# paLeziart/quadruped-reactive-walking

Hardware: AMD Instinct MI355X
Metric: control-steps/sec (MPC+WBC) (higher is better)
Workload: dtype f64

## Files before the change

### quadruped-reactive-walking_amd/csrc/chain_sweep.h

```cpp
#pragma once
#include <hip/hip_runtime.h>

#include "qrw_device.h"

namespace qrw {

constexpr int kCol = 14;
constexpr int kSlot = 168;
__host__ __device__ constexpr int chain_gap(int m) { return 0; }
__host__ __device__ constexpr int chain_slot(int slot, int m) { return slot * kSlot + (slot >= m ? chain_gap(m) : 0); }
__device__ __forceinline__ int chain_row_t(int lane) {
  const int l = lane & 15;
  return (l < 12) ? l : 11;
}
__host__ __device__ constexpr int chain_lds_doubles(int slots, int m) { return slots * kSlot + chain_gap(m); }

__device__ __forceinline__ double dpp_step12(double r, double x, const double (&m)[12]) {
  double a0 = r;
  asm("s_nop 1\n\t"
      "v_fmac_f64_dpp %0, %1, %2 row_newbcast:0 row_mask:0xf bank_mask:0xf\n\t"
      "v_fmac_f64_dpp %0, %1, %3 row_newbcast:1 row_mask:0xf bank_mask:0xf\n\t"
      "v_fmac_f64_dpp %0, %1, %4 row_newbcast:2 row_mask:0xf bank_mask:0xf\n\t"
      "v_fmac_f64_dpp %0, %1, %5 row_newbcast:3 row_mask:0xf bank_mask:0xf\n\t"
      "v_fmac_f64_dpp %0, %1, %6 row_newbcast:4 row_mask:0xf bank_mask:0xf\n\t"
      "v_fmac_f64_dpp %0, %1, %7 row_newbcast:5 row_mask:0xf bank_mask:0xf\n\t"
      "v_fmac_f64_dpp %0, %1, %8 row_newbcast:6 row_mask:0xf bank_mask:0xf\n\t"
      "v_fmac_f64_dpp %0, %1, %9 row_newbcast:7 row_mask:0xf bank_mask:0xf\n\t"
      "v_fmac_f64_dpp %0, %1, %10 row_newbcast:8 row_mask:0xf bank_mask:0xf\n\t"
      "v_fmac_f64_dpp %0, %1, %11 row_newbcast:9 row_mask:0xf bank_mask:0xf\n\t"
      "v_fmac_f64_dpp %0, %1, %12 row_newbcast:10 row_mask:0xf bank_mask:0xf\n\t"
      "v_fmac_f64_dpp %0, %1, %13 row_newbcast:11 row_mask:0xf bank_mask:0xf\n\t"
      : "+v"(a0)
      : "v"(x), "v"(m[0]), "v"(m[1]), "v"(m[2]), "v"(m[3]), "v"(m[4]), "v"(m[5]), "v"(m[6]), "v"(m[7]), "v"(m[8]),
        "v"(m[9]), "v"(m[10]), "v"(m[11]));
  return a0;
}

__host__ __device__ __forceinline__ int chain_pos(int k, int m, int N) { return (k <= m) ? k : m + N - k; }

struct ChainOp {
  double m[12];
  double r;
};
typedef double qrw_d2 __attribute__((ext_vector_type(2)));

__device__ __forceinline__ double swap_halves(double v) {
  int lo = __double2loint(v), hi = __double2hiint(v);
  asm("s_nop 1\n\tv_permlane32_swap_b32 %0, %0\n\tv_permlane32_swap_b32 %1, %1" : "+v"(lo), "+v"(hi));
  return __hiloint2double(hi, lo);
}

__device__ __forceinline__ double swap_rows16(double v) {
  int lo = __double2loint(v), hi = __double2hiint(v);
  asm("s_nop 1\n\tv_permlane16_swap_b32 %0, %0\n\tv_permlane16_swap_b32 %1, %1" : "+v"(lo), "+v"(hi));
  return __hiloint2double(hi, lo);
}

template <int NC>
__device__ __forceinline__ void chain_forward_paired(const double* sN, double* sX, double* sDump, int lane) {
  constexpr int N = NC, m = N >> 1, LA = m, LB = N - 1 - m, NP = LA / 2;
  static_assert(LA % 2 == 0 && LB == LA - 1, "paired sweeps need an even chain length");
  const int i = ((lane & 15) < 12) ? (lane & 15) : 11;
  const int h = lane >> 5;
  const bool rw = (lane & 16) != 0;
  const bool own = (lane & 15) < 12;
  const double* pm = sN + (rw ? m * kSlot + chain_gap(m) : 0) + h * kSlot + i;
  double* px = sX + (rw ? (m + 1) * 12 : 0) + i;
  const double* pr = px + h * 12;
  double* dump = sDump + i;
  double* ps_odd = (own && h == 1) ? px : dump;
  double* ps_even = (own && h == 0) ? px : dump;
  double* ps_oddA = (own && h == 1 && !rw) ? px : dump;
  double x = px[0], pB = 0.0;
  ChainOp b0, b1;
  auto fetch = [&](ChainOp& b, int p) {
    const double* q = pm + 2 * p * kSlot;
#pragma unroll
    for (int c = 0; c < 12; c++) b.m[c] = __hip_atomic_load(q + c * kCol, __ATOMIC_RELAXED, __HIP_MEMORY_SCOPE_WAVEFRONT);
    b.r = pr[(2 * p + 1) * 12];
  };
  auto pair = [&](const ChainOp& b, int p) {
    const int t1 = 2 * p + 1, t2 = t1 + 1;
    x = dpp_step12(b.r, x, b.m);
    x = swap_halves(x);
    if (t1 == LB) pB = x;
    (t1 < LB ? ps_odd : ps_oddA)[t1 * 12] = x;
    x = dpp_step12(b.r, x, b.m);
    if (t2 < LA) {
      x = swap_halves(x);
      ps_even[t2 * 12] = x;
    }
  };
  fetch(b0, 0);
#pragma unroll
  for (int p = 0; p < NP; p += 2) {
    if (p + 1 < NP) fetch(b1, p + 1);
    __builtin_amdgcn_sched_barrier(0);
    pair(b0, p);
    if (p + 1 < NP) {
      if (p + 2 < NP) fetch(b0, p + 2);
      __builtin_amdgcn_sched_barrier(0);
      pair(b1, p + 1);
    }
  }
  x += swap_rows16(pB);
  if (lane >= 32 && lane < 44) sX[m * 12 + i] = x;
}
template <int NC>
__device__ __forceinline__ void chain_backward_paired(const double* sN, double* sX, double* sDump, int lane) {
  constexpr int N = NC, m = N >> 1, LA = m, LB = N - 1 - m, NP = LA / 2;
  static_assert(LA % 2 == 0 && LB == LA - 1, "paired sweeps need an even chain length");
  const int i = ((lane & 15) < 12) ? (lane & 15) : 11;
  const int h = lane >> 5;
  const bool rw = (lane & 16) != 0;
  const bool own = (lane & 15) < 12;
  const int ib = chain_row_t(lane);
  const double* pm = sN + ((rw ? (N - 1) : m) - LA - h) * kSlot + (rw ? chain_gap(m) : 0) + ib * kCol;
  double* px = sX + ((rw ? N : m) - LA) * 12 + i;
  const double* pr = px - h * 12;
  double* dump = sDump + i;
  double* ps_odd = (own && h == 1) ? px : dump;
  double* ps_even = (own && h == 0) ? px : dump;
  double* ps_lastA = (own && h == 1 && !rw) ? px : dump;
  double x = sX[m * 12 + i];
  ChainOp b0, b1;
  auto fetch = [&](ChainOp& b, int p) {
    const qrw_d2* q = reinterpret_cast<const qrw_d2*>(pm + (LA - 2 * p - 1) * kSlot);
#pragma unroll
    for (int c = 0; c < 6; c++) {
      const qrw_d2 v = q[c];
      b.m[2 * c] = v.x;
      b.m[2 * c + 1] = v.y;
    }
    b.r = pr[(LA - 2 * p - 1) * 12];
  };
  auto pair = [&](const ChainOp& b, int p) {
    const int t1 = 2 * p + 1, t2 = t1 + 1;
    x = dpp_step12(b.r, x, b.m);
    x = swap_halves(x);
    ps_odd[(LA - t1) * 12] = x;
    x = dpp_step12(b.r, x, b.m);
    if (t2 < LA) {
      x = swap_halves(x);
      ps_even[(LA - t2) * 12] = x;
    } else {
      ps_lastA[(LA - t2) * 12] = x;
    }
  };
  fetch(b0, 0);
#pragma unroll
  for (int p = 0; p < NP; p += 2) {
    if (p + 1 < NP) fetch(b1, p + 1);
    __builtin_amdgcn_sched_barrier(0);
    pair(b0, p);
    if (p + 1 < NP) {
      if (p + 2 < NP) fetch(b0, p + 2);
      __builtin_amdgcn_sched_barrier(0);
      pair(b1, p + 1);
    }
  }
}

template <int NC>
__device__ __forceinline__ void chain_forward(const double* sN, double* sX, double* sDump, int Nrt, int lane) {
  if constexpr (NC > 0 && (NC / 2) % 2 == 0) {
    chain_forward_paired<NC>(sN, sX, sDump, lane);
    return;
  }
  const int N = NC ? NC : Nrt;
  const int m = N >> 1, LA = m, LB = N - 1 - m;
  if (LA == 0) return;
  asm volatile("" : "+v"(lane));
  const int i = ((lane & 15) < 12) ? (lane & 15) : 11;
  const bool rw = (lane & 16) != 0;
  const bool wr = (lane < 32) && ((lane & 15) < 12);
  const double* pm = sN + (rw ? m * kSlot + chain_gap(m) : 0) + i;
  double* px = sX + (rw ? (m + 1) * 12 : 0) + i;
  double* ps_early = wr ? px : sDump + i;
  double* ps_late = (wr && !rw) ? px : sDump + i;
  double x = px[0], pB = 0.0;
  ChainOp b0, b1;
  auto fetch = [&](ChainOp& b, int t) {
    const double* q = pm + (t - 1) * kSlot;
#pragma unroll
    for (int c = 0; c < 12; c++) {
      b.m[c] = __hip_atomic_load(q + c * kCol, __ATOMIC_RELAXED, __HIP_MEMORY_SCOPE_WAVEFRONT);
    }
    b.r = px[t * 12];
  };
  auto step = [&](const ChainOp& b, int t) {
    x = dpp_step12(b.r, x, b.m);
    if (t == LB) pB = x;
    if (t < LA) (t < LB ? ps_early : ps_late)[t * 12] = x;
  };
  fetch(b0, 1);
#pragma unroll
  for (int t = 1; t <= LA; t += 2) {
    if (t + 1 <= LA) fetch(b1, t + 1);
    __builtin_amdgcn_sched_barrier(0);
    step(b0, t);
    if (t + 1 <= LA) {
      if (t + 2 <= LA) fetch(b0, t + 2);
      __builtin_amdgcn_sched_barrier(0);
      step(b1, t + 1);
    }
  }
  if (LB > 0) x += shfl(pB, lane + 16);
  if (lane < 12) sX[m * 12 + i] = x;
}
template <int NC>
__device__ __forceinline__ void chain_backward(const double* sN, double* sX, double* sDump, int Nrt, int lane) {
  if constexpr (NC > 0 && (NC / 2) % 2 == 0) {
    chain_backward_paired<NC>(sN, sX, sDump, lane);
    return;
  }
  const int N = NC ? NC : Nrt;
  const int m = N >> 1, LA = m, LB = N - 1 - m;
  if (LA == 0) return;
  asm volatile("" : "+v"(lane));
  const int i = ((lane & 15) < 12) ? (lane & 15) : 11;
  const bool rw = (lane & 16) != 0;
  const bool wr = (lane < 32) && ((lane & 15) < 12);
  const int ib = chain_row_t(lane);
  const double* pm = sN + ((rw ? (N - 1) : m) - LA) * kSlot + (rw ? chain_gap(m) : 0) + ib * kCol;
  double* px = sX + ((rw ? N : m) - LA) * 12 + i;
  double* ps_early = wr ? px : sDump + i;
  double* ps_late = (wr && !rw) ? px : sDump + i;
  double x = sX[m * 12 + i];
  ChainOp b0, b1;
  auto fetch = [&](ChainOp& b, int t) {
    const qrw_d2* q = reinterpret_cast<const qrw_d2*>(pm + (LA - t) * kSlot);
#pragma unroll
    for (int c = 0; c < 6; c++) {
      const qrw_d2 v = q[c];
      b.m[2 * c] = v.x;
      b.m[2 * c + 1] = v.y;
    }
    b.r = px[(LA - t) * 12];
  };
  auto step = [&](const ChainOp& b, int t) {
    x = dpp_step12(b.r, x, b.m);
    (t <= LB ? ps_early : ps_late)[(LA - t) * 12] = x;
  };
  fetch(b0, 1);
#pragma unroll
  for (int t = 1; t <= LA; t += 2) {
    if (t + 1 <= LA) fetch(b1, t + 1);
    __builtin_amdgcn_sched_barrier(0);
    step(b0, t);
    if (t + 1 <= LA) {
      if (t + 2 <= LA) fetch(b0, t + 2);
      __builtin_amdgcn_sched_barrier(0);
      step(b1, t + 1);
    }
  }
}

#define QRW_GJ_FM(C) "v_fmac_f64_dpp %" #C ", %" #C ", %12 row_newbcast:%13 row_mask:0xf bank_mask:0xf\n\t"
template <int P>
__device__ __forceinline__ void gj_pivot(double (&m)[12], int i) {
  double piv = 0.0;
  const double one = 1.0;
  asm("s_nop 1\n\tv_fmac_f64_dpp %0, %1, %2 row_newbcast:%3 row_mask:0xf bank_mask:0xf" : "+v"(piv) : "v"(m[P]), "v"(one), "n"(P));
  const double d = fast_rcp(piv);
  const double f = (i == P) ? (d - 1.0) : (-m[P] * d);
  asm("s_nop 1\n\t" QRW_GJ_FM(0) QRW_GJ_FM(1) QRW_GJ_FM(2) QRW_GJ_FM(3) QRW_GJ_FM(4) QRW_GJ_FM(5) QRW_GJ_FM(6) QRW_GJ_FM(7)
      QRW_GJ_FM(8) QRW_GJ_FM(9) QRW_GJ_FM(10) QRW_GJ_FM(11)
      : "+v"(m[0]), "+v"(m[1]), "+v"(m[2]), "+v"(m[3]), "+v"(m[4]), "+v"(m[5]), "+v"(m[6]), "+v"(m[7]), "+v"(m[8]),
        "+v"(m[9]), "+v"(m[10]), "+v"(m[11])
      : "v"(f), "n"(P));
  m[P] = (i == P) ? d : f;
}
#undef QRW_GJ_FM
__device__ __forceinline__ void gj_invert12(double (&m)[12], int i) {
  gj_pivot<0>(m, i); gj_pivot<1>(m, i); gj_pivot<2>(m, i); gj_pivot<3>(m, i); gj_pivot<4>(m, i); gj_pivot<5>(m, i);
  gj_pivot<6>(m, i); gj_pivot<7>(m, i); gj_pivot<8>(m, i); gj_pivot<9>(m, i); gj_pivot<10>(m, i); gj_pivot<11>(m, i);
}
template <int J>
__device__ __forceinline__ void row_bcast_fma(double (&acc)[12], const double (&m)[12], double coef) {
  asm("s_nop 1\n\t"
      "v_fmac_f64_dpp %0, %12, %24 row_newbcast:%25 row_mask:0xf bank_mask:0xf\n\t"
      "v_fmac_f64_dpp %1, %13, %24 row_newbcast:%25 row_mask:0xf bank_mask:0xf\n\t"
      "v_fmac_f64_dpp %2, %14, %24 row_newbcast:%25 row_mask:0xf bank_mask:0xf\n\t"
      "v_fmac_f64_dpp %3, %15, %24 row_newbcast:%25 row_mask:0xf bank_mask:0xf\n\t"
      "v_fmac_f64_dpp %4, %16, %24 row_newbcast:%25 row_mask:0xf bank_mask:0xf\n\t"
      "v_fmac_f64_dpp %5, %17, %24 row_newbcast:%25 row_mask:0xf bank_mask:0xf\n\t"
      "v_fmac_f64_dpp %6, %18, %24 row_newbcast:%25 row_mask:0xf bank_mask:0xf\n\t"
      "v_fmac_f64_dpp %7, %19, %24 row_newbcast:%25 row_mask:0xf bank_mask:0xf\n\t"
      "v_fmac_f64_dpp %8, %20, %24 row_newbcast:%25 row_mask:0xf bank_mask:0xf\n\t"
      "v_fmac_f64_dpp %9, %21, %24 row_newbcast:%25 row_mask:0xf bank_mask:0xf\n\t"
      "v_fmac_f64_dpp %10, %22, %24 row_newbcast:%25 row_mask:0xf bank_mask:0xf\n\t"
      "v_fmac_f64_dpp %11, %23, %24 row_newbcast:%25 row_mask:0xf bank_mask:0xf\n\t"
      : "+v"(acc[0]), "+v"(acc[1]), "+v"(acc[2]), "+v"(acc[3]), "+v"(acc[4]), "+v"(acc[5]), "+v"(acc[6]), "+v"(acc[7]),
        "+v"(acc[8]), "+v"(acc[9]), "+v"(acc[10]), "+v"(acc[11])
      : "v"(m[0]), "v"(m[1]), "v"(m[2]), "v"(m[3]), "v"(m[4]), "v"(m[5]), "v"(m[6]), "v"(m[7]), "v"(m[8]), "v"(m[9]),
        "v"(m[10]), "v"(m[11]), "v"(coef), "n"(J));
}
__device__ __forceinline__ double row_shr6(double v) {
  int lo = __double2loint(v), hi = __double2hiint(v);
  lo = __builtin_amdgcn_update_dpp(0, lo, 0x116, 0xF, 0xF, false);
  hi = __builtin_amdgcn_update_dpp(0, hi, 0x116, 0xF, 0xF, false);
  return __hiloint2double(hi, lo);
}

}
```

### quadruped-reactive-walking_amd/csrc/mpc_kernel.hip

```cpp
#include <hip/hip_runtime.h>
#include <math.h>
#include <stdint.h>

#include <type_traits>
#include <vector>

#include "chain_sweep.h"
#include "qrw_device.h"
#include "qrw_kernels.h"

namespace qrw {

namespace {

constexpr int kMatSz = 144;
constexpr int kWSz = 36;

template <int NW>
struct alignas(16) MpcLdsT {
  static constexpr int S = 16 * NW;
  double sN[chain_lds_doubles(S, S / 2)];
  double sX[(S + 2) * 12];
  double sDump[(S / 2 + 2) * 12];
  double sE[S * 12];
// ... 1230 lines not shown
#ifdef QRW_TRACE_RES
        if (tid == 0 && a.prof && iter <= 4000) {
          double* tr = a.prof + (size_t)b * kMpcProfItems + (iter / 200 - 1) * 3;
          tr[0] = pri_res / (eps_abs + eps_rel * last_np); tr[1] = dua_res / (eps_abs + eps_rel * last_nd); tr[2] = rho;
        }
#endif
        if constexpr (PRE) {
          if (iter - it_resume >= a.pre_chunk && iter < max_iter) {
            if (pre_may_park<NW>(a, &L.sBal[0], tid)) parked = true;
            else it_resume = iter;
          }
          if (tid == 0) {
            double* pr = &L.sPre[(iter / 200 & 1) * 4];
            pr[0] = pri_res; pr[1] = last_np; pr[2] = dua_res; pr[3] = last_nd;
          }
        }
      }
      PH(7);
      if constexpr (PRE) {
        if (parked) break;
      }
    }
  }
  PH(7);
#ifdef QRW_PROFILE_PHASES
  if (tid == 0 && a.prof) for (int i = 0; i < 10; i++) a.prof[(size_t)b * kMpcProfItems + i] = (double)ph_acc[i];
#endif
  if (iter > max_iter) iter = max_iter;
  if (status == kStatusUnsolved && !parked) {
    const bool pok = pri_res < 10.0 * eps_abs + 10.0 * eps_rel * last_np;
    const bool dok = dua_res < 10.0 * eps_abs + 10.0 * eps_rel * last_nd;
    status = (pok && dok) ? kStatusSolvedInaccurate : kStatusMaxIter;
  }

  {
  QRW_UNPARK()
  const bool has_sol = (status != kStatusNonCvx);
  if (act && !parked) {
#pragma unroll
    for (int t = 0; t < 3; t++) {
      const int i = 3 * j + t;
      const double sx = has_sol ? xhX[t] + xr[i * (N + 1) + k + 1] : nan("");
      const double sf = has_sol ? xhF[t] : nan("");
      outp[i * N + k] = sx;
      outp[(12 + i) * N + k] = sf;
    }
  }
#pragma unroll
  for (int t = 0; t < 3; t++) {
    xX[t] = parked ? xhX[t] : xhX[t] * iDx[t]; xF[t] = parked ? xhF[t] : xhF[t] * iDf[t];
    zD[t] = Ed[t] * uD0[t];
    yD[t] = parked ? thD[t] : (thD[t] + zeU[t]) * (1.0 / Ed[t]);
    yS[t] = parked ? etS[t] : etS[t] * (1.0 / Es[t]);
  }
#pragma unroll
  for (int c = 0; c < 5; c++) {
    zC[c] = parked ? zeC[c] : zeC[c] * (1.0 / (rho_used * Ec[c]));
    yC[c] = parked ? etC[c] : etC[c] * (1.0 / Ec[c]);
  }
  if (!has_sol) {
#pragma unroll
    for (int t = 0; t < 3; t++) xX[t] = xF[t] = zD[t] = yD[t] = yS[t] = 0.0;
#pragma unroll
    for (int c = 0; c < 5; c++) zC[c] = yC[c] = 0.0;
  }
  ST(kStRho) = rho;
  ST(kStC) = parked ? rho_used : cs;
#pragma unroll
  for (int t = 0; t < 3; t++) {
    ST(kStXX + t) = xX[t]; ST(kStXF + t) = xF[t]; ST(kStZD + t) = zD[t];
    ST(kStYD + t) = yD[t]; ST(kStYS + t) = yS[t]; ST(kStS + t) = sfl[t];
    ST(kStDX + t) = 1.0 / iDx[t]; ST(kStDF + t) = 1.0 / iDf[t]; ST(kStED + t) = Ed[t]; ST(kStES + t) = Es[t];
#pragma unroll
    for (int r = 0; r < 3; r++) ST(kStB + r * 3 + t) = Bang[r][t];
  }
#pragma unroll
  for (int c = 0; c < 5; c++) { ST(kStZC + c) = zC[c]; ST(kStYC + c) = yC[c]; ST(kStEC + c) = Ec[c]; }
  if (PRE && parked) {
    if (tid == 0) {
      a.pause_it[b] = iter;
      a.rho_updates[b] = rho_updates;
    }
  } else if (tid == 0) {
    if constexpr (PRE) a.pause_it[b] = 0;
    a.flags[b] = 1;
    a.iters[b] = iter;
    a.status[b] = status;
    a.rho_out[b] = rho;
    a.pri[b] = pri_res;
    a.dua[b] = dua_res;
    a.rho_updates[b] = rho_updates;
    if (SEQ && a.seq_iters) a.seq_iters[io] = iter;
#ifdef QRW_SEQ_STATS
    if (a.prof && a.seq_K <= 5) {
      a.prof[io * 2] = (double)(__builtin_amdgcn_s_memrealtime() - task_t0);
      a.prof[io * 2 + 1] = (double)iter;
    }
#endif
  }
  }
  }
  if constexpr (SEQ) seq_finish_task<NW>(a, b, seq_s, tid);
  if constexpr (PRE) {
    int level = 0;
    if (parked && tid == 0) {
      const int it = a.pause_it[b];
      const double* p1 = &L.sPre[(it / 200 & 1) * 4];
      const double* p0 = &L.sPre[((it / 200 & 1) ^ 1) * 4];
      const double r1 = fmax(p1[0] / (1e-6 + 1e-6 * p1[1]), p1[2] / (1e-6 + 1e-6 * p1[3]));
      const double r0 = (p0[1] > 0.0 || p0[3] > 0.0) ? fmax(p0[0] / (1e-6 + 1e-6 * p0[1]), p0[2] / (1e-6 + 1e-6 * p0[3])) : 0.0;
      level = pre_level(a, it, it_resume, r1, r0);
    }
    pre_end_chunk<NW>(a, b, parked, level, tid);
  }
  }
#undef QRW_UNPARK
#undef ST
}

namespace {
__device__ __forceinline__ int order_key(float e) {
  const int key = (int)(e * 0.04f);
  return key < 0 ? 0 : (key > 160 ? 160 : key);
}
__device__ __forceinline__ float order_ema(float e0, float it) { return (e0 == 0.0f) ? it : e0 + (it - e0) * 0.125f; }
}

__global__ __launch_bounds__(64) void mpc_order_kernel(const int* __restrict__ iters, float* __restrict__ ema,
                                                       int* __restrict__ order, int B) {
  constexpr int U = 4, R = 64 * 4 * U;
  __shared__ int hist[162];
  __shared__ int offs[162];
  const int lane = threadIdx.x;
  for (int i = lane; i < 162; i += 64) hist[i] = 0;
  __syncthreads();
  const int Bv = B - B % R;
  for (int base = 0; base < Bv; base += R) {
    int4 it[U];
    float4 e[U];
#pragma unroll
    for (int u = 0; u < U; u++) {
      const int b = base + (u * 64 + lane) * 4;
      it[u] = *reinterpret_cast<const int4*>(iters + b);
      e[u] = *reinterpret_cast<const float4*>(ema + b);
    }
#pragma unroll
    for (int u = 0; u < U; u++) {
      const int b = base + (u * 64 + lane) * 4;
      e[u].x = order_ema(e[u].x, (float)it[u].x);
      e[u].y = order_ema(e[u].y, (float)it[u].y);
      e[u].z = order_ema(e[u].z, (float)it[u].z);
      e[u].w = order_ema(e[u].w, (float)it[u].w);
      *reinterpret_cast<float4*>(ema + b) = e[u];
      atomicAdd(&hist[order_key(e[u].x)], 1);
      atomicAdd(&hist[order_key(e[u].y)], 1);
      atomicAdd(&hist[order_key(e[u].z)], 1);
      atomicAdd(&hist[order_key(e[u].w)], 1);
    }
  }
  for (int b = Bv + lane; b < B; b += 64) {
    const float e = order_ema(ema[b], (float)iters[b]);
    ema[b] = e;
    atomicAdd(&hist[order_key(e)], 1);
  }
  __syncthreads();
  {
    const int k0 = 160 - 3 * lane;
    int h[3], tot = 0;
#pragma unroll
    for (int j = 0; j < 3; j++) { h[j] = (k0 - j >= 0) ? hist[k0 - j] : 0; tot += h[j]; }
    int incl = tot;
#pragma unroll
    for (int d = 1; d < 64; d <<= 1) {
      const int up = __shfl_up(incl, d, 64);
      if (lane >= d) incl += up;
    }
    int run = incl - tot;
#pragma unroll
    for (int j = 0; j < 3; j++) { if (k0 - j >= 0) offs[k0 - j] = run; run += h[j]; }
  }
  __syncthreads();
  for (int base = 0; base < Bv; base += R) {
    float4 e[U];
#pragma unroll
    for (int u = 0; u < U; u++) e[u] = *reinterpret_cast<const float4*>(ema + base + (u * 64 + lane) * 4);
#pragma unroll
    for (int u = 0; u < U; u++) {
      const int b = base + (u * 64 + lane) * 4;
      order[atomicAdd(&offs[order_key(e[u].x)], 1)] = b;
      order[atomicAdd(&offs[order_key(e[u].y)], 1)] = b + 1;
      order[atomicAdd(&offs[order_key(e[u].z)], 1)] = b + 2;
      order[atomicAdd(&offs[order_key(e[u].w)], 1)] = b + 3;
    }
  }
  for (int b = Bv + lane; b < B; b += 64) order[atomicAdd(&offs[order_key(ema[b])], 1)] = b;
}

int mpc_order_launch(const int* iters, float* ema, int* order, int B, hipStream_t stream) {
  hipLaunchKernelGGL(mpc_order_kernel, dim3(1), dim3(64), 0, stream, iters, ema, order, B);
  return hipGetLastError() == hipSuccess ? 0 : -2;
}

int mpc_preemptive_launch(const MpcArgs& a_in, int resident_slots, hipStream_t stream) {
  if (a_in.N <= 16 || a_in.N > kMpcMaxN || !a_in.pre_queue || !a_in.pre_ctr || !a_in.pause_it || a_in.pre_chunk < 200 || a_in.pre_cmax < 1 ||
      a_in.pre_levels < 1 || a_in.pre_levels > kPreMaxLevels || a_in.pre_bin < 1) return -1;
  MpcArgs a = a_in;
  auto go = [&](unsigned blocks) {
    if (a.N == 32) hipLaunchKernelGGL((mpc_solve_kernel<2, true, false, true>), dim3(blocks), dim3(128), 0, stream, a);
    else hipLaunchKernelGGL((mpc_solve_kernel<2, false, false, true>), dim3(blocks), dim3(128), 0, stream, a);
  };
  const unsigned takers = (unsigned)a.B * (unsigned)(a.pre_cmax - 1);
  if (a.B > resident_slots || takers == 0u) {
    a.pre_block0 = 0;
    go((unsigned)a.B + takers);
  } else {
    a.pre_block0 = 0;
    go((unsigned)a.B);
    a.pre_block0 = a.B;
    go(takers);
  }
  return hipGetLastError() == hipSuccess ? 0 : -2;
}

__global__ void mpc_pre_error_flush_kernel(const unsigned* pre_ctr, unsigned* host_word) {
  const unsigned code = pre_ctr[kPreErr];
  if (code != 0u) __hip_atomic_store(host_word, code, __ATOMIC_RELAXED, __HIP_MEMORY_SCOPE_SYSTEM);
}
int mpc_pre_error_flush(const unsigned* pre_ctr, unsigned* host_word, hipStream_t stream) {
  hipLaunchKernelGGL(mpc_pre_error_flush_kernel, dim3(1), dim3(1), 0, stream, pre_ctr, host_word);
  return hipGetLastError() == hipSuccess ? 0 : -2;
}

int mpc_launch(const MpcArgs& a, hipStream_t stream) {
  if (a.N < 1 || a.N > kMpcMaxN) return -1;
  if (a.N == 16) hipLaunchKernelGGL((mpc_solve_kernel<1, true, false>), dim3(a.B), dim3(64), 0, stream, a);
  else if (a.N < 16) hipLaunchKernelGGL((mpc_solve_kernel<1, false, false>), dim3(a.B), dim3(64), 0, stream, a);
  else if (a.N == 32) hipLaunchKernelGGL((mpc_solve_kernel<2, true, false>), dim3(a.B), dim3(128), 0, stream, a);
  else hipLaunchKernelGGL((mpc_solve_kernel<2, false, false>), dim3(a.B), dim3(128), 0, stream, a);
  return hipGetLastError() == hipSuccess ? 0 : -2;
}

__global__ void mpc_seq_init_kernel(int* queue, unsigned* qctr, int* level, int* first, const int* order, int B, int K, int groups) {
  __shared__ unsigned n_lvl[kSeqLevels], base[kSeqLevels], n_q[kSeqLevels], n_dealt[kSeqLevels];
  const int cut[kSeqLevels] = {B / 16, B / 4, B / 2, B};
  auto level_of = [&](int rank) {
    if (!order) return kSeqLevels - 1;
    for (int l = 0; l < kSeqLevels; l++) if (rank < cut[l]) return l;
    return kSeqLevels - 1;
  };
  if (threadIdx.x == 0) {
    unsigned run = 0;
    for (int l = 0; l < kSeqLevels; l++) {
      const int lo = (l == 0) ? 0 : cut[l - 1];
      n_lvl[l] = order ? (unsigned)(cut[l] - lo) : (l == kSeqLevels - 1 ? (unsigned)B : 0u);
      base[l] = run;
      run += n_lvl[l] * (unsigned)K;
      n_q[l] = 0;
      n_dealt[l] = 0;
    }
  }
  __syncthreads();
  for (long i = threadIdx.x; i < (long)B * K; i += blockDim.x) queue[i] = -1;
  __syncthreads();
  for (int r = threadIdx.x; r < B; r += blockDim.x) {
    const int b = order ? order[r] : r;
    const int l = level_of(r);
    level[b] = l;
    if (r < groups) first[r] = b;
  }
  __syncthreads();
  if (threadIdx.x == 0) {
    for (int r = 0; r < B; r++) {
      const int l = level_of(r);
      if (r < groups) n_dealt[l]++;
      else queue[base[l] + n_q[l]++] = order ? order[r] : r;
    }
    for (int l = 0; l < kSeqLevels; l++) {
      qctr[l * kSeqStride] = 0u;
      qctr[l * kSeqStride + 1] = n_q[l];
      qctr[kSeqErr + 2 + l] = n_lvl[l] * (unsigned)K - n_dealt[l];
      qctr[kSeqErr + 16 + l] = base[l];
    }
    qctr[kSeqErr] = 0u;
    qctr[kSeqErr + 1] = 0u;
    qctr[kSeqProgress] = 0u;
  }
}

int mpc_sequence_launch(const MpcArgs& a, hipStream_t stream) {
  if (a.N < 1 || a.N > kMpcMaxN || a.seq_K < 1 || !a.queue || !a.qctr || !a.seq_hot || !a.seq_first || a.seq_groups < 1) return -1;
  hipLaunchKernelGGL(mpc_seq_init_kernel, dim3(1), dim3(1024), 0, stream, a.queue, a.qctr, a.seq_hot, a.seq_first, a.order, a.B, a.seq_K,
                     a.seq_groups);
  const unsigned tasks = (unsigned)a.seq_K * (unsigned)a.B;
  if (a.N == 16) hipLaunchKernelGGL((mpc_solve_kernel<1, true, true>), dim3(tasks), dim3(64), 0, stream, a);
  else if (a.N < 16) hipLaunchKernelGGL((mpc_solve_kernel<1, false, true>), dim3(tasks), dim3(64), 0, stream, a);
  else if (a.N == 32) hipLaunchKernelGGL((mpc_solve_kernel<2, true, true>), dim3(tasks), dim3(128), 0, stream, a);
  else hipLaunchKernelGGL((mpc_solve_kernel<2, false, true>), dim3(tasks), dim3(128), 0, stream, a);
  return hipGetLastError() == hipSuccess ? 0 : -2;
}

}

namespace qrw {
__global__ void sweeps_selftest_kernel(const double* M, const double* r, const double* G, double* out, double* ginv) {
  __shared__ __attribute__((aligned(16))) double sN[chain_lds_doubles(16, 8)];
  __shared__ double sX[18 * 12];
  __shared__ double sDump[10 * 12];
  const int lane = threadIdx.x;
  for (int e = lane; e < chain_lds_doubles(16, 8); e += 64) sN[e] = M[e];
  for (int e = lane; e < 18 * 12; e += 64) sX[e] = r[e];
  __syncthreads();
  chain_forward<16>(sN, sX, sDump, 16, lane);
  __syncthreads();
  chain_backward<16>(sN, sX, sDump, 16, lane);
  __syncthreads();
  for (int e = lane; e < 18 * 12; e += 64) out[e] = sX[e];
  const int i = ((lane & 15) < 12) ? (lane & 15) : 11, which = (lane >> 4) & 1;
  double m[12];
#pragma unroll
  for (int c = 0; c < 12; c++) m[c] = G[which * 144 + i * 12 + c];
  gj_invert12(m, i);
  if (lane < 32 && (lane & 15) < 12)
#pragma unroll
    for (int c = 0; c < 12; c++) ginv[which * 144 + i * 12 + c] = m[c];
}

namespace {
struct SelfTestBuf {
  void* p = nullptr;
  ~SelfTestBuf() { if (p) hipFree(p); }
  bool alloc(size_t bytes) { return hipMalloc(&p, bytes) == hipSuccess; }
  template <typename T> T* as() const { return static_cast<T*>(p); }
};
struct SelfTestStream {
  hipStream_t s = nullptr;
  ~SelfTestStream() { if (s) hipStreamDestroy(s); }
  bool create() { return hipStreamCreateWithFlags(&s, hipStreamNonBlocking) == hipSuccess; }
};
}

int sweeps_selftest(double* max_err) {
  constexpr int N = 16, m = N / 2;
  std::vector<double> hMv(chain_lds_doubles(16, 8), 0.0), hrv(18 * 12), houtv(18 * 12), hGv(288), hGiv(288);
  double *hM = hMv.data(), *hr = hrv.data(), *hout = houtv.data(), *hG = hGv.data(), *hGi = hGiv.data();
  for (int s = 0; s < N - 1; s++)
    for (int i = 0; i < 12; i++)
      for (int c = 0; c < 12; c++) hM[chain_slot(s, m) + c * kCol + i] = 0.25 * sin(0.37 * (s * 144 + i * 12 + c) + 1.0);
  for (int e = 0; e < 18 * 12; e++) hr[e] = 0.0;
  for (int k = 0; k < N; k++)
    for (int i = 0; i < 12; i++) hr[chain_pos(k, m, N) * 12 + i] = cos(0.11 * (k * 12 + i));
  for (int w = 0; w < 2; w++)
    for (int i = 0; i < 12; i++)
      for (int c = 0; c < 12; c++) hG[w * 144 + i * 12 + c] = ((i == c) ? 4.0 + w : 0.0) + 0.3 * sin(1.7 * (w * 144 + i * 12 + c));
  auto Mat = [&](int slot, int i, int c) { return hM[chain_slot(slot, m) + c * kCol + i]; };
  double u[N][12], t[12];
  for (int k = 0; k < N; k++) for (int i = 0; i < 12; i++) u[k][i] = hr[chain_pos(k, m, N) * 12 + i];
  for (int k = 1; k < m; k++) for (int i = 0; i < 12; i++) { double s = u[k][i]; for (int c = 0; c < 12; c++) s += Mat(k - 1, i, c) * u[k - 1][c]; u[k][i] = s; }
  for (int k = N - 2; k > m; k--) { for (int i = 0; i < 12; i++) { double s = u[k][i]; for (int c = 0; c < 12; c++) s += Mat(m + N - 2 - k, i, c) * u[k + 1][c]; t[i] = s; } for (int i = 0; i < 12; i++) u[k][i] = t[i]; }
  for (int i = 0; i < 12; i++) { double s = u[m][i], s2 = 0; for (int c = 0; c < 12; c++) { s += Mat(m - 1, i, c) * u[m - 1][c]; s2 += Mat(N - 2, i, c) * u[m + 1][c]; } t[i] = s + s2; }
  for (int i = 0; i < 12; i++) u[m][i] = t[i];
  for (int k = m - 1; k >= 0; k--) { for (int i = 0; i < 12; i++) { double s = u[k][i]; for (int c = 0; c < 12; c++) s += Mat(k, c, i) * u[k + 1][c]; t[i] = s; } for (int i = 0; i < 12; i++) u[k][i] = t[i]; }
  for (int k = m + 1; k < N; k++) { for (int i = 0; i < 12; i++) { double s = u[k][i]; for (int c = 0; c < 12; c++) s += Mat(m + N - 2 - (k - 1), c, i) * u[k - 1][c]; t[i] = s; } for (int i = 0; i < 12; i++) u[k][i] = t[i]; }
  SelfTestBuf bM, br, bG, bout, bGi;
  SelfTestStream st;
  const size_t nM = hMv.size() * sizeof(double), nr = hrv.size() * sizeof(double), nG = hGv.size() * sizeof(double);
  if (!bM.alloc(nM) || !br.alloc(nr) || !bG.alloc(nG) || !bout.alloc(nr) || !bGi.alloc(nG) || !st.create()) return -1;
  hipMemcpyAsync(bM.p, hM, nM, hipMemcpyHostToDevice, st.s); hipMemcpyAsync(br.p, hr, nr, hipMemcpyHostToDevice, st.s);
  hipMemcpyAsync(bG.p, hG, nG, hipMemcpyHostToDevice, st.s);
  hipLaunchKernelGGL(sweeps_selftest_kernel, dim3(1), dim3(64), 0, st.s, bM.as<double>(), br.as<double>(), bG.as<double>(), bout.as<double>(),
                     bGi.as<double>());
  hipMemcpyAsync(hout, bout.p, nr, hipMemcpyDeviceToHost, st.s); hipMemcpyAsync(hGi, bGi.p, nG, hipMemcpyDeviceToHost, st.s);
  if (hipStreamSynchronize(st.s) != hipSuccess) return -2;
  double me = 0.0;
  for (int k = 0; k < N; k++) for (int i = 0; i < 12; i++) me = fmax(me, fabs(hout[chain_pos(k, m, N) * 12 + i] - u[k][i]) / 8.0);
  for (int w = 0; w < 2; w++)
    for (int i = 0; i < 12; i++)
      for (int c = 0; c < 12; c++) {
        double s = 0.0;
        for (int q = 0; q < 12; q++) s += hG[w * 144 + i * 12 + q] * hGi[w * 144 + q * 12 + c];
        me = fmax(me, fabs(s - ((i == c) ? 1.0 : 0.0)));
      }
  if (max_err) *max_err = me;
  return (me < 1e-12) ? 0 : 1;
}
}
```

Baseline: 685,100.

## Add quad-split chain sweeps using both wavefront halves for long horizons

Adds forward and backward chain-sweep variants for horizons whose half-length is a multiple of 4, used for N=32. They split each step pair across the two 32-lane halves of the wavefront, passing the running vector between halves with swap_halves so all 64 lanes carry work. The intent is to shorten the serial dependent DPP FMA chain and hide LDS fetch latency. It adds cross-half swaps, extra dump-slot stores, and more intricate indexing. The self-test is templated so N=32 gets checked as well.

```diff
diff --git a/quadruped-reactive-walking_amd/csrc/chain_sweep.h b/quadruped-reactive-walking_amd/csrc/chain_sweep.h
--- a/quadruped-reactive-walking_amd/csrc/chain_sweep.h
+++ b/quadruped-reactive-walking_amd/csrc/chain_sweep.h
@@ -162,7 +162,114 @@
 }
 
 template <int NC>
+__device__ __forceinline__ void chain_forward_quad(const double* sN, double* sX, double* sDump, int lane) {
+  constexpr int N = NC, m = N >> 1, LA = m, LB = N - 1 - m, NQ = LA / 4;
+  static_assert(LA % 4 == 0 && LB == LA - 1, "the 2 + 2 half order needs a chain length that is a multiple of 4");
+  const int i = ((lane & 15) < 12) ? (lane & 15) : 11;
+  const int h = lane >> 5;
+  const bool rw = (lane & 16) != 0;
+  const bool own = (lane & 15) < 12;
+  const double* pm = sN + (rw ? m * kSlot + chain_gap(m) : 0) + 2 * h * kSlot + i;
+  double* px = sX + (rw ? (m + 1) * 12 : 0) + i;
+  const double* pr = px + 2 * h * 12;
+  double* dump = sDump + i;
+  double* ps_lo = (own && h == 0) ? px : dump;
+  double* ps_hi = (own && h == 1) ? px : dump;
+  double* ps_hiA = (own && h == 1 && !rw) ? px : dump;
+  double x = px[0], pB = 0.0;
+  ChainOp bX, bY;
+  auto fetch = [&](ChainOp& b, int s) {
+    const double* q = pm + s * kSlot;
+#pragma unroll
+    for (int c = 0; c < 12; c++) b.m[c] = __hip_atomic_load(q + c * kCol, __ATOMIC_RELAXED, __HIP_MEMORY_SCOPE_WAVEFRONT);
+    b.r = pr[(s + 1) * 12];
+  };
+  fetch(bX, 0);
+  fetch(bY, 1);
+#pragma unroll
+  for (int q = 0; q < NQ; q++) {
+    const int t = 4 * q;
+    __builtin_amdgcn_sched_barrier(0);
+    x = dpp_step12(bX.r, x, bX.m);
+    ps_lo[(t + 1) * 12] = x;
+    x = dpp_step12(bY.r, x, bY.m);
+    x = swap_halves(x);
+    ps_hi[(t + 2) * 12] = x;
+    x = dpp_step12(bX.r, x, bX.m);
+    if (t + 3 == LB) pB = x;
+    (t + 3 < LB ? ps_hi : ps_hiA)[(t + 3) * 12] = x;
+    if (q + 1 < NQ) fetch(bX, t + 4);
+    __builtin_amdgcn_sched_barrier(0);
+    x = dpp_step12(bY.r, x, bY.m);
+    if (q + 1 < NQ) {
+      x = swap_halves(x);
+      ps_lo[(t + 4) * 12] = x;
+      fetch(bY, t + 5);
+    }
+  }
+  x += swap_rows16(pB);
+  if (lane >= 32 && lane < 44) sX[m * 12 + i] = x;
+}
+template <int NC>
+__device__ __forceinline__ void chain_backward_quad(const double* sN, double* sX, double* sDump, int lane) {
+  constexpr int N = NC, m = N >> 1, LA = m, LB = N - 1 - m, NQ = LA / 4;
+  static_assert(LA % 4 == 0 && LB == LA - 1, "the 2 + 2 half order needs a chain length that is a multiple of 4");
+  const int i = ((lane & 15) < 12) ? (lane & 15) : 11;
+  const int h = lane >> 5;
+  const bool rw = (lane & 16) != 0;
+  const bool own = (lane & 15) < 12;
+  const int ib = chain_row_t(lane);
+  const double* pm = sN + ((rw ? (N - 1) : m) - LA - 2 * h) * kSlot + (rw ? chain_gap(m) : 0) + ib * kCol;
+  double* px = sX + ((rw ? N : m) - LA) * 12 + i;
+  const double* pr = px - 2 * h * 12;
+  double* dump = sDump + i;
+  double* ps_lo = (own && h == 0) ? px : dump;
+  double* ps_hi = (own && h == 1) ? px : dump;
+  double* ps_lastA = (own && h == 1 && !rw) ? px : dump;
+  double x = sX[m * 12 + i];
+  ChainOp bX, bY;
+  auto fetch = [&](ChainOp& b, int t) {
+    const qrw_d2* q = reinterpret_cast<const qrw_d2*>(pm + (LA - t) * kSlot);
+#pragma unroll
+    for (int c = 0; c < 6; c++) {
+      const qrw_d2 v = q[c];
+      b.m[2 * c] = v.x;
+      b.m[2 * c + 1] = v.y;
+    }
+    b.r = pr[(LA - t) * 12];
+  };
+  fetch(bX, 1);
+  fetch(bY, 2);
+#pragma unroll
+  for (int q = 0; q < NQ; q++) {
+    const int t = 4 * q;
+    __builtin_amdgcn_sched_barrier(0);
+    x = dpp_step12(bX.r, x, bX.m);
+    ps_lo[(LA - t - 1) * 12] = x;
+    x = dpp_step12(bY.r, x, bY.m);
+    x = swap_halves(x);
+    ps_hi[(LA - t - 2) * 12] = x;
+    x = dpp_step12(bX.r, x, bX.m);
+    ps_hi[(LA - t - 3) * 12] = x;
+    if (q + 1 < NQ) fetch(bX, t + 5);
+    __builtin_amdgcn_sched_barrier(0);
+    x = dpp_step12(bY.r, x, bY.m);
+    if (q + 1 < NQ) {
+      x = swap_halves(x);
+      ps_lo[(LA - t - 4) * 12] = x;
+      fetch(bY, t + 6);
+    } else {
+      ps_lastA[0] = x;
+    }
+  }
+}
+
+template <int NC>
 __device__ __forceinline__ void chain_forward(const double* sN, double* sX, double* sDump, int Nrt, int lane) {
+  if constexpr (NC > 0 && (NC / 2) % 4 == 0) {
+    chain_forward_quad<NC>(sN, sX, sDump, lane);
+    return;
+  }
   if constexpr (NC > 0 && (NC / 2) % 2 == 0) {
     chain_forward_paired<NC>(sN, sX, sDump, lane);
     return;
@@ -210,6 +317,10 @@
 }
 template <int NC>
 __device__ __forceinline__ void chain_backward(const double* sN, double* sX, double* sDump, int Nrt, int lane) {
+  if constexpr (NC > 0 && (NC / 2) % 4 == 0) {
+    chain_backward_quad<NC>(sN, sX, sDump, lane);
+    return;
+  }
   if constexpr (NC > 0 && (NC / 2) % 2 == 0) {
     chain_backward_paired<NC>(sN, sX, sDump, lane);
     return;
diff --git a/quadruped-reactive-walking_amd/csrc/mpc_kernel.hip b/quadruped-reactive-walking_amd/csrc/mpc_kernel.hip
--- a/quadruped-reactive-walking_amd/csrc/mpc_kernel.hip
+++ b/quadruped-reactive-walking_amd/csrc/mpc_kernel.hip
@@ -1556,27 +1556,30 @@
 }
 
 namespace qrw {
+template <int NC>
 __global__ void sweeps_selftest_kernel(const double* M, const double* r, const double* G, double* out, double* ginv) {
-  __shared__ __attribute__((aligned(16))) double sN[chain_lds_doubles(16, 8)];
-  __shared__ double sX[18 * 12];
-  __shared__ double sDump[10 * 12];
+  __shared__ __attribute__((aligned(16))) double sN[chain_lds_doubles(NC, NC / 2)];
+  __shared__ double sX[(NC + 2) * 12];
+  __shared__ double sDump[(NC / 2 + 2) * 12];
   const int lane = threadIdx.x;
-  for (int e = lane; e < chain_lds_doubles(16, 8); e += 64) sN[e] = M[e];
-  for (int e = lane; e < 18 * 12; e += 64) sX[e] = r[e];
+  for (int e = lane; e < chain_lds_doubles(NC, NC / 2); e += 64) sN[e] = M[e];
+  for (int e = lane; e < (NC + 2) * 12; e += 64) sX[e] = r[e];
   __syncthreads();
-  chain_forward<16>(sN, sX, sDump, 16, lane);
+  chain_forward<NC>(sN, sX, sDump, NC, lane);
   __syncthreads();
-  chain_backward<16>(sN, sX, sDump, 16, lane);
+  chain_backward<NC>(sN, sX, sDump, NC, lane);
   __syncthreads();
-  for (int e = lane; e < 18 * 12; e += 64) out[e] = sX[e];
-  const int i = ((lane & 15) < 12) ? (lane & 15) : 11, which = (lane >> 4) & 1;
-  double m[12];
-#pragma unroll
-  for (int c = 0; c < 12; c++) m[c] = G[which * 144 + i * 12 + c];
-  gj_invert12(m, i);
-  if (lane < 32 && (lane & 15) < 12)
-#pragma unroll
-    for (int c = 0; c < 12; c++) ginv[which * 144 + i * 12 + c] = m[c];
+  for (int e = lane; e < (NC + 2) * 12; e += 64) out[e] = sX[e];
+  if constexpr (NC == 16) {
+    const int i = ((lane & 15) < 12) ? (lane & 15) : 11, which = (lane >> 4) & 1;
+    double m[12];
+#pragma unroll
+    for (int c = 0; c < 12; c++) m[c] = G[which * 144 + i * 12 + c];
+    gj_invert12(m, i);
+    if (lane < 32 && (lane & 15) < 12)
+#pragma unroll
+      for (int c = 0; c < 12; c++) ginv[which * 144 + i * 12 + c] = m[c];
+  }
 }
 
 namespace {
@@ -1593,14 +1596,27 @@
 };
 }
 
+template <int N>
+static int sweeps_selftest_n(double* max_err);
+
 int sweeps_selftest(double* max_err) {
-  constexpr int N = 16, m = N / 2;
-  std::vector<double> hMv(chain_lds_doubles(16, 8), 0.0), hrv(18 * 12), houtv(18 * 12), hGv(288), hGiv(288);
+  double e16 = 0.0, e32 = 0.0;
+  const int rc16 = sweeps_selftest_n<16>(&e16);
+  const int rc32 = (rc16 < 0) ? rc16 : sweeps_selftest_n<32>(&e32);
+  if (max_err) *max_err = fmax(e16, e32);
+  if (rc16 < 0 || rc32 < 0) return rc16 < 0 ? rc16 : rc32;
+  return (rc16 || rc32) ? 1 : 0;
+}
+
+template <int N>
+static int sweeps_selftest_n(double* max_err) {
+  constexpr int m = N / 2;
+  std::vector<double> hMv(chain_lds_doubles(N, m), 0.0), hrv((N + 2) * 12), houtv((N + 2) * 12), hGv(288), hGiv(288);
   double *hM = hMv.data(), *hr = hrv.data(), *hout = houtv.data(), *hG = hGv.data(), *hGi = hGiv.data();
   for (int s = 0; s < N - 1; s++)
     for (int i = 0; i < 12; i++)
       for (int c = 0; c < 12; c++) hM[chain_slot(s, m) + c * kCol + i] = 0.25 * sin(0.37 * (s * 144 + i * 12 + c) + 1.0);
-  for (int e = 0; e < 18 * 12; e++) hr[e] = 0.0;
+  for (int e = 0; e < (N + 2) * 12; e++) hr[e] = 0.0;
   for (int k = 0; k < N; k++)
     for (int i = 0; i < 12; i++) hr[chain_pos(k, m, N) * 12 + i] = cos(0.11 * (k * 12 + i));
   for (int w = 0; w < 2; w++)
@@ -1621,13 +1637,13 @@
   if (!bM.alloc(nM) || !br.alloc(nr) || !bG.alloc(nG) || !bout.alloc(nr) || !bGi.alloc(nG) || !st.create()) return -1;
   hipMemcpyAsync(bM.p, hM, nM, hipMemcpyHostToDevice, st.s); hipMemcpyAsync(br.p, hr, nr, hipMemcpyHostToDevice, st.s);
   hipMemcpyAsync(bG.p, hG, nG, hipMemcpyHostToDevice, st.s);
-  hipLaunchKernelGGL(sweeps_selftest_kernel, dim3(1), dim3(64), 0, st.s, bM.as<double>(), br.as<double>(), bG.as<double>(), bout.as<double>(),
+  hipLaunchKernelGGL(sweeps_selftest_kernel<N>, dim3(1), dim3(64), 0, st.s, bM.as<double>(), br.as<double>(), bG.as<double>(), bout.as<double>(),
                      bGi.as<double>());
   hipMemcpyAsync(hout, bout.p, nr, hipMemcpyDeviceToHost, st.s); hipMemcpyAsync(hGi, bGi.p, nG, hipMemcpyDeviceToHost, st.s);
   if (hipStreamSynchronize(st.s) != hipSuccess) return -2;
   double me = 0.0;
   for (int k = 0; k < N; k++) for (int i = 0; i < 12; i++) me = fmax(me, fabs(hout[chain_pos(k, m, N) * 12 + i] - u[k][i]) / 8.0);
-  for (int w = 0; w < 2; w++)
+  for (int w = 0; w < (N == 16 ? 2 : 0); w++)
     for (int i = 0; i < 12; i++)
       for (int c = 0; c < 12; c++) {
         double s = 0.0;
```

After: 701,700, median of 6. 2.4% higher.
